# facebookresearch/holo_diffusion

Measured on AMD Instinct MI355X. Metric: denoise-steps/sec + rendered-rays/sec, 64^3x32 grid @400^2 render, higher is better.
Workload: dtype f32

## Files before the change

### holo_diffusion_amd/csrc/conv_weights.h

```cpp
#pragma once
#include <stddef.h>
#include <stdint.h>

#include "holo_knobs.h"

namespace holo {

int64_t conv_wino3_weight_floats(int CoutP, int CinP, int src_taps);

inline int64_t round64(int64_t n) { return (n + 63) & ~(int64_t)63; }

inline int conv_cout_tile(int Cout) { return Cout >= 64 ? 64 : 32; }
struct ConvWeightLayout {
  int Cout = 0, Cin = 0, taps = 0;
  int CoutP = 0, CinP = 0;
  int64_t f32_floats() const { return (int64_t)taps * CoutP * CinP; }
  int64_t bf16_elems() const { return 4 * round64(f32_floats()); }
  int64_t bft_offset() const { return 3 * f32_floats(); }
  int64_t wino2_floats() const { return (int64_t)(taps == 27 ? 48 : 4) * CoutP * CinP; }
  int64_t wino3_floats() const { return conv_wino3_weight_floats(CoutP, CinP, taps); }
};
inline ConvWeightLayout conv_weight_layout(int Cout, int Cin, int taps) {
  const int tile = conv_cout_tile(Cout);
  return {Cout, Cin, taps, (Cout + tile - 1) / tile * tile, (Cin + 31) / 32 * 32};
}

struct ConvCopies {
  bool bf16 = false, wino2 = false, wino3 = false;
};
inline ConvCopies forward_copies(const ConvWeightLayout& l, bool skip, const Knobs& k) {
  ConvCopies c;
  const bool c3 = l.taps == 27;
  c.bf16 = true;
  c.wino2 = k.conv_wino != 0 && (c3 || skip) && l.Cout <= 256 && l.Cin <= 768 && (l.Cout % 64 == 0 || (c3 && l.Cout == 32));
  c.wino3 = c.wino2 && k.conv_wino3 != 0 && l.Cout % 64 == 0;
  return c;
}
inline ConvCopies dgrad_copies(const ConvWeightLayout& l, int compute_mode, const Knobs& k) {
  ConvCopies c;
  c.wino2 = k.conv_wino != 0 && compute_mode == 0 && l.taps == 27 && l.Cout % 64 == 0 && l.Cout <= 768 && l.Cin <= 768;
  c.wino3 = c.wino2 && k.conv_wino3 != 0 && l.Cout <= 256;
  return c;
}

struct ConvWeights {
  float* f32 = nullptr;
  uint16_t* bf = nullptr;
  uint16_t* bft = nullptr;
  float* wino2 = nullptr;
  float* wino3 = nullptr;
  ConvWeightLayout layout;
};
int pack_conv_weights(const float* src_oidhw, const ConvWeights& dst, void* stream);

}
```

### holo_diffusion_amd/csrc/holo_kernels.h

```cpp
#pragma once
#include <stddef.h>
#include <stdint.h>

#include "../../include/holo_abi.h"
#include "conv_weights.h"
#include "holo_knobs.h"

struct HoloCtx {
  int device;
  int num_cus;
  int deterministic = 0;
};

namespace holo {

enum class ConvKernel : int32_t {
  Gather = 0,
  Halo = 1,
  RowTile = 2,
  Wino2 = 4,
  Bf16Wide = 5,
  Wino3 = 6,
  Stream1x1 = 7,
  Bf16Persistent = 8,
  S2Bf16 = 9,
  Qkv = 10,
  Bf16Stream1x1 = 11,
  Small1x1 = 12,
};

struct ConvParams {
  const float* src0;
  const float* src1;
  int C0, C1;
  int N, ID, IH, IW;
  int ups;
  int OD, OH, OW;
  int stride, pad, ksz;
  int Cout;
  const float* w;
  int CoutP, CinP;
  const float* coef;
  int act;
  const float* bias;
  const float* residual;
  float* out;
  const float* skip_src0;
  const float* skip_src1;
  int skip_C0, skip_C1;
  const float* skip_w;
  const uint16_t* w_bf;
// ... 11 lines not shown
  int stagger_ticks;
  unsigned long long* dbg;
  ConvKernel kernel;
  const float* w_wino2;
  const float* skip_w_wino2;
  const float* w_wino3;
  const float* skip_w_wino3;
  int wino3_up;
  const uint16_t* w_bft;
  const uint16_t* skip_w_bft;
  int in_bf16;
  int res_bf16;
  int out_bf16;
  uint16_t* qkv_q;
  uint16_t* qkv_k;
  uint16_t* qkv_vt;
  float qkv_scale;
  int qkv_T, qkv_CH, qkv_H;
  int qkv_sb, qkv_rows;
};

bool conv_s2_bf16_supported(const ConvParams& p);
int conv_s2_bf16_launch(const ConvParams& p, void* stream);

bool conv1x1_qkv_bf16_supported(const ConvParams& p);
void conv1x1_qkv_bf16_plan(ConvParams& p, int num_cus);
int conv1x1_qkv_bf16_launch(const ConvParams& p, void* stream);
bool conv1x1_bf16_stream_supported(const ConvParams& p);
void conv1x1_bf16_stream_plan(ConvParams& p, int num_cus);
int conv1x1_bf16_stream_slabs(const ConvParams& p);
int conv1x1_bf16_stream_launch(const ConvParams& p, void* stream);

int repack_conv_weight_wino3_launch(const float* w, float* out, int Cout, int Cin, int src_taps, int CoutP, int CinP,
                                    void* stream);
int conv_wino3_launch(const ConvParams& p, void* stream);
int conv_bf16p_launch(const ConvParams& p, void* stream);

size_t conv_plan(ConvParams& p, int num_cus, const Knobs& k, int plan_n = 0);
int conv_launch(const ConvParams& p, void* stream);
int conv_stats_slabs(const ConvParams& p);
double conv_flops(const ConvParams& p);
double conv_exec_flops(const ConvParams& p);

struct GemmParams {
  const float* A;
  const float* B;
// ... 395 lines not shown
```

### holo_diffusion_amd/csrc/holo_knobs.h

```cpp
#pragma once

#include <stdint.h>
#include <stdlib.h>

namespace holo {

#ifdef HOLO_EMU
constexpr bool EMU_BUILD = true;
#else
constexpr bool EMU_BUILD = false;
#endif

constexpr int64_t KNOB_UNSET = INT64_MIN;

#define HOLO_KNOBS(X)                                                                                                      \
  X(num_cus, "HOLO_NUM_CUS", POS, 0, CTX, "planners size grids and split-K for this many CUs (default: the device's)")     \
  X(conv_wino, "HOLO_CONV_WINO", INT, 1, HANDLE, "0: no Winograd copies of the conv weights (forward and dgrad)")          \
  X(conv_wino3, "HOLO_CONV_WINO3", INT, 1, HANDLE_PLAN, "0: no F(2x2x2, 3x3x3) copies / conv_wino3_kernel never chosen")   \
  X(keep_intermediates, "HOLO_KEEP_INTERMEDIATES", CH, '1', HANDLE,                                                        \
    "1: the plan releases no activation, holo_unet_fetch_block works")                                                     \
  X(render_v1, "HOLO_RENDER_V1", SET, 0, HANDLE, "the ray-per-column render kernel for everything")                        \
  X(render2_nw, "HOLO_RENDER2_NW", INT, 0, HANDLE, "8: the 8-wave form of render2_kernel's 12-wave configurations")        \
  X(render2_nrm_nw, "HOLO_RENDER2_NRM_NW", INT, 0, HANDLE,                                                                 \
    "8: rendered normals two waves per SIMD instead of 10 waves (the emulation build always runs 8)")                      \
  X(render_wgs, "HOLO_RENDER_WGS", POS, 0, HANDLE, "persistent render workgroups (default: one per CU)")                   \
  X(render_xcd, "HOLO_RENDER_XCD", RAW, KNOB_UNSET, HANDLE,                                                                \
    "XCD ranges of the render tile order (default 8; 2 in the emulation build; <= 1: plain order)")                        \
  X(render_tail, "HOLO_RENDER_TAIL", RAW, KNOB_UNSET, HANDLE,                                                              \
    "4-ray tiles at the end of every XCD range handed out as single rays (default: about two rounds; 3 in the "            \
    "emulation build; 0: off)")                                                                                            \
  X(render_static_tiles, "HOLO_RENDER_STATIC_TILES", SET, 0, HANDLE, "static tile stride instead of the dynamic hand-out") \
  X(render_timeline, "HOLO_RENDER_TIMELINE", SET, 0, HANDLE, "per-phase clocks of every render launch (synchronises!)")    \
  X(mlp_mean_bwd_chunk, "HOLO_MLP_MEAN_BWD_CHUNK", POS, 0, HANDLE,                                                         \
    "voxels per chunk of holo_mlp_mean_backward (default: what fits 4 GiB of rows; the emulation build: always 2048)")     \
  X(conv_wino_small, "HOLO_CONV_WINO_SMALL", INT, 1, PLAN, "0: under-filled levels take 64-voxel tiles, not Winograd")     \
  X(conv_force_tz2, "HOLO_CONV_FORCE_TZ2", INT, 0, PLAN, "1: 128-voxel tiles (hence the Winograd kernels) on small grids") \
  X(conv_qkv_fused, "HOLO_CONV_QKV_FUSED", INT, 1, PLAN, "0: row-tile qkv convolution + attn_pack_kernel")                 \
  X(conv1x1_bf16_stream, "HOLO_CONV1X1_BF16_STREAM", INT, 1, PLAN, "0: the row-tile kernel for bf16 1x1x1 convolutions")   \
  X(conv1x1_stream_min_m, "HOLO_CONV1X1_STREAM_MIN_M", INT, 131072, PLAN,                                                  \
    "rows from which a raw-input fp32 1x1x1 convolution streams (0: never)")                                               \
  X(conv1x1_small, "HOLO_CONV1X1_SMALL", INT, 1, PLAN, "0: the row-tile kernel for the fp32 attention's 1x1x1 convs")      \
  X(conv_s2t, "HOLO_CONV_S2T", INT, -1, PLAN, "stride-2 bf16 halo kernel: 0 never, 1 wherever defined (default: by fill)") \
  X(conv_bf16t, "HOLO_CONV_BF16T", INT, -1, PLAN, "bf16 wide-tile kernel: 0 never, 1 everywhere (default: by fill / K)")   \
  X(conv_bf16p, "HOLO_CONV_BF16P", INT, -1, PLAN,                                                                          \
    "its persistent form: 0 never, 1 every wide-tile launch, 2 activated input too (default: raw input)")                  \
  X(conv_bf16p_wgs, "HOLO_CONV_BF16P_WGS", INT, 0, PLAN, "at most this many persistent workgroups (0: no cap)")            \
  X(conv_wino3_min_items, "HOLO_CONV_WINO3_MIN_ITEMS", INT, KNOB_UNSET, PLAN,                                              \
    "work items from which conv_wino3_kernel runs (default: num_cus / 2)")                                                 \
  X(conv_wino3_up, "HOLO_CONV_WINO3_UP", INT, 1, PLAN,                                                                     \
    "0: upsampling convolutions on conv_wino3_kernel's generic form (64 pseudo-taps), not its 27-tap form")               \
  X(no_skip_fusion, "HOLO_NO_SKIP_FUSION", SET, 0, PLAN, "a ResBlock's 1x1x1 skip always as its own launch")               \
  X(skip_fusion_below_r, "HOLO_SKIP_FUSION_BELOW_R", RAW, 64, PLAN,                                                        \
    "exact fp32: the skip is fused into the second convolution below this grid edge")                                      \
  X(no_flash_attn, "HOLO_NO_FLASH_ATTN", SET, 0, PLAN, "attention as GEMM + softmax + GEMM")                               \
  X(bf16_flash_min_t, "HOLO_BF16_FLASH_MIN_T", RAW, 1024, PLAN, "tokens from which the bf16 mode takes its bf16 attention") \
  X(flash_split, "HOLO_FLASH_SPLIT", INT, 0, PLAN, "key splits of the fp32 attention, clamped to [1, T/128] (0: by fill)") \
  X(flash_v2_ksplit, "HOLO_FLASH_V2_KSPLIT", INT, 0, PLAN,                                                                 \
    "key splits of the bf16 attention: 1..8 dividing T into multiples of 128, else ignored")                               \
  X(attn_exact, "HOLO_ATTN_EXACT", SET, 0, PLAN, "bf16 attention: the exact loop alone, no LAZY pass")                     \
  X(debug_timestep_load, "HOLO_DEBUG_TIMESTEP_LOAD", INT, 0, PLAN, "how time_embed_kernel loads the timesteps (see it)")   \
  X(dgrad_s2_direct, "HOLO_DGRAD_S2_DIRECT", CH, '1', PLAN, "1: conv_dgrad_s2_kernel for every Downsample dgrad")          \
  X(wgrad_tiles, "HOLO_WGRAD_TILES", POS, 0, PLAN, "> 0: the tile weight-gradient kernel instead of the row-staged one")   \
  X(wgrad_reduce_tile_min, "HOLO_WGRAD_REDUCE_TILE_MIN", RAW, 1024, PLAN,                                                  \
    "64-element tiles from which the weight-gradient reduce runs its tile form")                                           \
  X(debug_plan, "HOLO_DEBUG_PLAN", SET, 0, PLAN, "[plan] lines on stderr: what every convolution / attention launches")    \
// ... 35 lines not shown
```

### holo_diffusion_amd/csrc/kernels_conv.hip

```cpp
#include <stdio.h>
#include <stdlib.h>

#include "holo_common.h"
#include "holo_kernels.h"

namespace holo {

namespace {

constexpr int BM = 128;
constexpr int BK = 32;
constexpr int LDK = 36;

__device__ __forceinline__ float silu_f(float v) { return v / (1.0f + __expf(-v)); }
__device__ __forceinline__ float silu_fast(float v) { return v * holo_rcp(1.0f + __expf(-v)); }

__device__ __forceinline__ float bf16_load(const uint16_t* p) { return __uint_as_float((uint32_t)(*p) << 16); }
__device__ __forceinline__ uint16_t bf16_round(float v) { return (uint16_t)(pack_bf16x2(v, 0.f) & 0xffffu); }
__device__ __forceinline__ float4 ld_act4(const float* base, int64_t idx, int bf) {
  if (bf) {
    const uint2 u = *reinterpret_cast<const uint2*>(reinterpret_cast<const uint16_t*>(base) + idx);
    return make_float4(__uint_as_float(u.x << 16), __uint_as_float(u.x & 0xffff0000u), __uint_as_float(u.y << 16),
                       __uint_as_float(u.y & 0xffff0000u));
  }
// ... 2230 lines not shown
    double* dst = stats + (((int64_t)n * gridDim.x + blockIdx.x) * Cout + c_base + tid * 4) * 2;
#pragma unroll
    for (int e = 0; e < 4; ++e) {
      dst[e * 2 + 0] = s[e];
      dst[e * 2 + 1] = s[4 + e];
    }
  }
}

const char* conv_kernel_name(ConvKernel k) {
  switch (k) {
    case ConvKernel::Gather: return "conv_igemm_kernel";
    case ConvKernel::Halo: return "conv_halo_kernel";
    case ConvKernel::RowTile: return "conv_small_kernel";
    case ConvKernel::Wino2: return "conv_wino2_kernel";
    case ConvKernel::Bf16Wide: return "conv_bf16t_kernel";
    case ConvKernel::Wino3: return "conv_wino3_kernel";
    case ConvKernel::Stream1x1: return "conv1x1_stream_kernel";
    case ConvKernel::Bf16Persistent: return "conv_bf16p_kernel";
    case ConvKernel::S2Bf16: return "conv_s2_bf16_kernel";
    case ConvKernel::Qkv: return "conv1x1_qkv_bf16_kernel";
    case ConvKernel::Bf16Stream1x1: return "conv1x1_bf16_stream_kernel";
    case ConvKernel::Small1x1: return "conv1x1_small_kernel";
  }
  return "?";
}

constexpr int SM_SPLIT_WGS_PER_CU = 2;
constexpr int BF16T_LONG_K = 192;
constexpr int BF16T_SPLIT_WGS_PER_CU_TOP = 2;
constexpr int BF16T_SPLIT_WGS_PER_CU = 1;

struct KSplit {
  int n, cps;
};
KSplit ksplit(int64_t want, int max_split, int chunks) {
  const int cps = (int)cdiv(chunks, want < max_split ? want : max_split);
  return {(int)cdiv(chunks, cps), cps};
}

bool conv1x1_small_supported(const ConvParams& p) {
  const int Cin = p.C0 + p.C1;
  const int64_t V = (int64_t)p.OD * p.OH * p.OW;
  return p.ksz == 1 && p.stride == 1 && p.pad == 0 && !p.ups && p.bf16 == 0 && !p.in_bf16 && !p.out_bf16 && !p.res_bf16 &&
         !p.skip_w && !p.src1 && p.C1 == 0 && !p.qkv_q && ((p.coef && !p.act) || p.residual) && (Cin % 32) == 0 &&
         Cin >= 32 && Cin <= 256 && p.CinP == Cin && (p.Cout % 64) == 0 && p.CoutP == p.Cout && p.ID == p.OD &&
// ... 11 lines not shown

size_t conv_plan(ConvParams& p, int num_cus, const Knobs& k, int plan_n) {
  const int Cin = p.C0 + p.C1;
  const int ncc = (Cin + BK - 1) / BK;
  const int nchunks = p.ksz * p.ksz * p.ksz * ncc;
  const int nsk = p.skip_w ? (int)cdiv(p.skip_C0 + p.skip_C1, BK) : 0;
  const int ncc16 = (Cin + 15) / 16;
  const int nsk16 = p.skip_w ? (p.skip_C0 + p.skip_C1 + 15) / 16 : 0;
  const int64_t M = (int64_t)p.N * p.OD * p.OH * p.OW;
  const int64_t Mc = (int64_t)(plan_n > 0 ? plan_n : p.N) * p.OD * p.OH * p.OW;
  const int bn = p.Cout >= 64 ? 64 : 32;
  const int64_t tiles = cdiv(Mc, BM) * cdiv(p.Cout, bn);
  const int64_t t8 = (Mc / 512) * cdiv(p.Cout, bn);
  const int64_t t3 = (Mc / 128) * (p.Cout / 64);
  const int64_t target = 2 * (int64_t)num_cus;
  const int64_t src_vox = (int64_t)p.ID * p.IH * p.IW;
  const int cmax = p.C0 > p.C1 ? p.C0 : p.C1;
  const int skmax = p.skip_C0 > p.skip_C1 ? p.skip_C0 : p.skip_C1;
  const bool fits32 = src_vox * (cmax > skmax ? cmax : skmax) * 4 < ((int64_t)1 << 32) &&
                      (int64_t)p.OD * p.OH * p.OW * p.Cout * 4 < ((int64_t)1 << 32);
  const bool halo = p.ksz == 3 && p.stride == 1 && p.pad == 1 && (p.OD % 2) == 0 && (p.OH % 8) == 0 && (p.OW % 8) == 0 &&
                    p.ID == p.OD && p.IH == p.OH && p.IW == p.OW && (Cin % 16) == 0 && fits32;
  const bool wino2_wide = p.w_wino2 && p.bf16 == 0 && p.Cout >= 64 && (p.Cout % 64) == 0 && (!p.skip_w || p.skip_w_wino2);
  const bool wino_small = k.conv_wino_small != 0 && wino2_wide && ncc >= 2;
  const int tz = tiles < target && k.conv_force_tz2 != 1 && !wino_small ? 1 : 2;

  const ConvKernel kernel = [&] {
    if (p.qkv_q) {
      if (k.conv_qkv_fused != 0 && conv1x1_qkv_bf16_supported(p)) return ConvKernel::Qkv;
      p.qkv_q = nullptr;
    }
    if (k.conv1x1_bf16_stream != 0 && conv1x1_bf16_stream_supported(p)) return ConvKernel::Bf16Stream1x1;
    if (!halo) {
      const int64_t min_m = k.conv1x1_stream_min_m;
      if (min_m > 0 && Mc >= min_m && p.ksz == 1 && p.stride == 1 && !p.ups && !p.coef && !p.residual && !p.skip_w && p.bf16 == 0 &&
          !p.in_bf16 && !p.out_bf16 && (p.Cout % 64) == 0 && (Cin % 32) == 0 && Cin >= 32 && Cin <= 256 &&
          (!p.src1 || (p.C0 % 32) == 0) && (Mc % 16) == 0 && p.ID == p.OD && p.IH == p.OH && p.IW == p.OW)
        return ConvKernel::Stream1x1;
      if (k.conv1x1_small != 0 && conv1x1_small_supported(p)) return ConvKernel::Small1x1;
      const int64_t s2t = k.conv_s2t;
      if (s2t != 0 && conv_s2_bf16_supported(p) && ((Mc / 128) * (p.Cout / 64) >= num_cus / 4 || s2t == 1))
        return ConvKernel::S2Bf16;
      return p.Cout >= 64 ? ConvKernel::RowTile : ConvKernel::Gather;
    }
    const int64_t bt = k.conv_bf16t;
    if (p.bf16 == 1 && p.in_bf16 && p.w_bft && (!p.skip_w || p.skip_w_bft) && (p.OD % 8) == 0 && (p.OH % 8) == 0 &&
        (p.OW % 8) == 0 && (p.Cout % 32) == 0 && (p.C0 % 8) == 0 && (p.skip_C0 % 8) == 0 && ((p.skip_C0 + p.skip_C1) % 8) == 0 &&
        (p.Cout >= 64 || !p.skip_w) && bt != 0 &&
        (t8 >= target || Cin + (p.skip_w ? p.skip_C0 + p.skip_C1 : 0) >= BF16T_LONG_K || bt == 1)) {
      const int64_t bp = k.conv_bf16p;
      const int wgs = num_cus & ~7;
      if (bp != 0 && (bp == 1 || bp == 2 || !p.coef) &&
          ((bf16t_split(p, t8, ncc16, num_cus).n == 1 && wgs >= 8 && t8 >= wgs) || bp == 1) &&
          (p.C1 == 0 || (p.C0 % 16) == 0) &&
          (!p.skip_w || (((p.skip_C0 + p.skip_C1) % 32) == 0 && (p.skip_C1 == 0 || (p.skip_C0 % 32) == 0))) &&
          src_vox < ((int64_t)1 << 24))
        return ConvKernel::Bf16Persistent;
      return ConvKernel::Bf16Wide;
    }
    if (tz == 2 && k.conv_wino3 != 0 && p.w_wino3 && p.bf16 == 0 && !p.in_bf16 && !p.out_bf16 && p.Cout >= 64 &&
        (p.Cout % 64) == 0 && (!p.skip_w || p.skip_w_wino3) && (p.OH % 8) == 0 && (p.OW % 8) == 0 && (p.OD % 2) == 0 &&
        (!p.coef || p.act) &&
        (int64_t)p.N * src_vox * (cmax > skmax ? cmax : skmax) * 4 < ((int64_t)1 << 32) &&
        (int64_t)wino3_split(t3, ncc, num_cus).n * Mc * p.Cout * 4 < ((int64_t)1 << 32) &&
        (!p.stats || (Mc / 128) * p.Cout * 16 < ((int64_t)1 << 32)) &&
        (!p.skip_w || ((p.skip_C0 % 16) == 0 && (p.skip_C1 % 4) == 0)) &&
        t3 * wino3_split(t3, ncc, num_cus).n >= (k.conv_wino3_min_items != KNOB_UNSET ? k.conv_wino3_min_items : num_cus / 2))
      return ConvKernel::Wino3;
    if (tz == 2 && (wino2_wide || (p.w_wino2 && p.bf16 == 0 && p.Cout == 32 && !p.skip_w))) return ConvKernel::Wino2;
    return ConvKernel::Halo;
  }();
  p.kernel = kernel;
  p.wino3_up = kernel == ConvKernel::Wino3 && p.ups && !p.coef && !p.skip_w && k.conv_wino3_up != 0 ? 1 : 0;

  switch (kernel) {
    case ConvKernel::Qkv:
    case ConvKernel::Bf16Stream1x1:
    case ConvKernel::Stream1x1:
    case ConvKernel::Small1x1:
      p.nsplit = 1;
      p.chunks_per_split = ncc;
      if (kernel == ConvKernel::Qkv) conv1x1_qkv_bf16_plan(p, num_cus);
      if (kernel == ConvKernel::Bf16Stream1x1) conv1x1_bf16_stream_plan(p, num_cus);
      break;
    case ConvKernel::S2Bf16:
      p.nsplit = 1;
      p.chunks_per_split = Cin / 16;
      break;
    case ConvKernel::RowTile: {
      const int64_t t2 = cdiv(Mc, SM_ROWS) * cdiv(p.Cout, 64);
      const int64_t tgt = SM_SPLIT_WGS_PER_CU * (int64_t)num_cus;
      const int nall = nchunks + nsk;
      const int max_split = nall / SG > 1 ? nall / SG : 1;
      const KSplit s = ksplit(t2 < tgt ? cdiv(tgt, t2) : 1, max_split, nall);
      p.nsplit = s.n;
      p.chunks_per_split = s.cps;
      break;
    }
    case ConvKernel::Gather: {
      const int max_split = nchunks / 4 > 1 ? nchunks / 4 : 1;
      const KSplit s = ksplit(tiles < target ? cdiv(target, tiles) : 1, max_split, nchunks);
      p.nsplit = s.n;
      p.chunks_per_split = s.cps;
      break;
    }
    case ConvKernel::Bf16Wide: {
      const KSplit s = bf16t_split(p, t8, ncc16, num_cus);
      p.tz = 8;
// ... 47 lines not shown
}

int conv_stats_slabs(const ConvParams& p) {
  const int64_t V = (int64_t)p.OD * p.OH * p.OW;
  if (p.nsplit > 1) {
    int B, vpb;
    gn_stats_geometry(p.Cout < 1024 ? p.Cout : 1024, V, &B, &vpb);
    return B;
  }
  switch (p.kernel) {
    case ConvKernel::Bf16Wide:
    case ConvKernel::Bf16Persistent:
      return (int)(V / 512);
    case ConvKernel::Halo:
      if (p.bf16 == 2 && p.w_bf && p.Cout >= 64 && !p.skip_w) return (int)(V / 32);
      [[fallthrough]];
    case ConvKernel::Wino2:
    case ConvKernel::Wino3:
      return (int)(V / (64 * p.tz)) * (p.Cout >= 64 ? 1 : 2);
    case ConvKernel::RowTile:
      return V % SM_ROWS == 0 ? (int)(V / SM_ROWS) : 0;
    case ConvKernel::S2Bf16:
      return (int)(V / 128);
    case ConvKernel::Bf16Stream1x1:
      return conv1x1_bf16_stream_slabs(p);
    case ConvKernel::Small1x1:
      return (int)(V / 16);
    default:
      return 0;
  }
}

double conv_flops(const ConvParams& p) {
  const double M = (double)p.N * p.OD * p.OH * p.OW;
  return 2.0 * M * p.Cout * ((double)(p.C0 + p.C1) * p.ksz * p.ksz * p.ksz + (p.skip_w ? p.skip_C0 + p.skip_C1 : 0));
}

double conv_exec_flops(const ConvParams& p) {
  const double wino3_taps = p.wino3_up ? 27.0 / 8.0 : 8.0;
  const double taps = p.kernel == ConvKernel::Wino3 ? wino3_taps : p.kernel == ConvKernel::Wino2 ? 12.0 : 0.0;
  if (taps == 0.0) return conv_flops(p);
  const double M = (double)p.N * p.OD * p.OH * p.OW;
  return 2.0 * M * p.Cout * ((double)(p.C0 + p.C1) * taps + (p.skip_w ? p.skip_C0 + p.skip_C1 : 0));
}

int conv_launch(const ConvParams& p, void* stream) {
// ... 137 lines not shown
      }
      dim3 g1((unsigned)(M / 16), (unsigned)(p.Cout / 64));
      switch (Cin / 32) {
        case 1: HOLO_LAUNCH(conv1x1_small_kernel<1>, g1, block, stream, p); break;
        case 2: HOLO_LAUNCH(conv1x1_small_kernel<2>, g1, block, stream, p); break;
        case 3: HOLO_LAUNCH(conv1x1_small_kernel<3>, g1, block, stream, p); break;
        case 4: HOLO_LAUNCH(conv1x1_small_kernel<4>, g1, block, stream, p); break;
        case 5: HOLO_LAUNCH(conv1x1_small_kernel<5>, g1, block, stream, p); break;
        case 6: HOLO_LAUNCH(conv1x1_small_kernel<6>, g1, block, stream, p); break;
        case 7: HOLO_LAUNCH(conv1x1_small_kernel<7>, g1, block, stream, p); break;
        case 8: HOLO_LAUNCH(conv1x1_small_kernel<8>, g1, block, stream, p); break;
        default:
          set_error("conv_launch: conv1x1_small_kernel: %d input channels", Cin);
          return -1;
      }
      break;
    }
    case ConvKernel::Bf16Persistent:
      if (conv_bf16p_launch(p, stream)) return -1;
      break;
    case ConvKernel::S2Bf16:
      if (conv_s2_bf16_launch(p, stream)) return -1;
      break;
    case ConvKernel::Qkv:
      if (conv1x1_qkv_bf16_launch(p, stream)) return -1;
      break;
    case ConvKernel::Bf16Stream1x1:
      if (conv1x1_bf16_stream_launch(p, stream)) return -1;
      break;
    default:
      set_error("conv_launch: unknown kernel %d", (int)p.kernel);
      return -1;
  }
  if (p.nsplit > 1) {
    const int64_t MC = M * p.Cout;
    const int64_t V = (int64_t)p.OD * p.OH * p.OW;
    int B, vpb;
    gn_stats_geometry(p.Cout < 1024 ? p.Cout : 1024, V, &B, &vpb);
    HOLO_LAUNCH(splitk_reduce_kernel, dim3((unsigned)B, (unsigned)p.N, (unsigned)cdiv(p.Cout, 1024)), dim3(256), stream,
                (const float*)p.partial,
                p.nsplit, MC, p.Cout, V, vpb, p.bias, p.skip_bias, p.residual, p.out, p.stats, p.res_bf16, p.out_bf16);
  }
  return 0;
}

}
// ... 1 lines not shown
```

### holo_diffusion_amd/csrc/kernels_conv_s2.hip

```cpp
#include "holo_common.h"
#include "holo_kernels.h"

namespace holo {
namespace {

constexpr int S2_HZ = 5, S2_HY = 17, S2_HX = 17, S2_XH = 9;
constexpr int S2_SLOTS = S2_HZ * S2_HY * 2 * S2_XH;
constexpr int S2_NV = S2_HZ * S2_HY * S2_HX;
constexpr int S2_IT = (2 * S2_NV + 255) / 256;

__global__ __launch_bounds__(256, 3) void conv_s2_bf16_kernel(ConvParams p) {
  __shared__ __attribute__((aligned(16))) float s_in[S2_SLOTS * 8];
  __shared__ float s_st[4 * 32 * 2];
  const int tid = threadIdx.x;
  const int lane = tid & 63;
  const int wave = tid >> 6;
  const int li = lane & 31;
  const int kg = lane >> 5;
  const int zw = wave >> 1;
  const int ch = wave & 1;
  const int Cin = p.C0;
  const int ncc = Cin / 16;
  const int ntx = p.OW >> 3, nty = p.OH >> 3, ntz = p.OD >> 1;
  int bt = blockIdx.x;
// ... 126 lines not shown
}

}

bool conv_s2_bf16_supported(const ConvParams& p) {
  const int Cin = p.C0 + p.C1;
  return p.ksz == 3 && p.stride == 2 && p.pad == 1 && !p.ups && p.bf16 == 1 && p.in_bf16 && p.out_bf16 && p.w_bft && !p.coef &&
         !p.residual && !p.skip_w && p.C1 == 0 && (Cin % 16) == 0 && (p.Cout % 64) == 0 && p.ID == 2 * p.OD && p.IH == 2 * p.OH &&
         p.IW == 2 * p.OW && (p.OD % 2) == 0 && (p.OH % 8) == 0 && (p.OW % 8) == 0 &&
         (int64_t)p.ID * p.IH * p.IW * Cin < ((int64_t)1 << 31);
}

int conv_s2_bf16_launch(const ConvParams& p, void* stream) {
  if (!conv_s2_bf16_supported(p) || p.nsplit != 1) {
    set_error("conv_s2_bf16_launch: unsupported launch (stride %d, %d -> %d channels, %d^3 -> %d^3)", p.stride, p.C0 + p.C1, p.Cout,
              p.ID, p.OD);
    return -1;
  }
  const int64_t tiles = (int64_t)p.N * (p.OD >> 1) * (p.OH >> 3) * (p.OW >> 3);
  HOLO_LAUNCH(conv_s2_bf16_kernel, dim3((unsigned)tiles, (unsigned)(p.Cout / 64)), dim3(256), stream, p);
  return 0;
}

}
```

### holo_diffusion_amd/csrc/unet_exec.cpp

```cpp
#include <math.h>
#include <stdarg.h>
#include <stdio.h>
#include <stdlib.h>
#include <string.h>

#include <functional>
#include <map>
#include <optional>
#include <string>
#include <vector>

#include "../../include/holo_abi.h"
#include "conv_weights.h"
#include "holo_common.h"
#include "holo_kernels.h"

namespace holo {

static thread_local char g_err[512] = "";
void set_error(const char* fmt, ...) {
  va_list ap;
  va_start(ap, fmt);
  vsnprintf(g_err, sizeof(g_err), fmt, ap);
  va_end(ap);
// ... 21 lines not shown
  if (!rc && dst.wino3) rc = repack_conv_weight_wino3_launch(src, dst.wino3, l.Cout, l.Cin, l.taps, l.CoutP, l.CinP, stream);
  return rc;
}


namespace {

enum BlockKind { B_CONV, B_RES, B_ATTN, B_DOWN, B_UP, B_HEAD };
struct Block {
  BlockKind kind;
  std::string prefix;
  int cin, cout;
};

enum ParamKind { P_PLAIN, P_CONV3, P_CONV1, P_EMB_W, P_EMB_B };

struct ParamSlot {
  std::string name;
  std::vector<int64_t> shape;
  int64_t numel;
  ParamKind kind;
  ConvWeights w;
  bool set;
  bool is_conv() const { return kind == P_CONV3 || kind == P_CONV1; }
  ConvWeightLayout layout(bool transposed = false) const {
    return conv_weight_layout((int)shape[transposed ? 1 : 0], (int)shape[transposed ? 0 : 1], kind == P_CONV3 ? 27 : 1);
  }
};
static bool is_downsample_weight(const std::string& name) {
  return name.size() > 10 && name.compare(name.size() - 10, 10, ".op.weight") == 0;
}

struct Arena {
  size_t top = 0, peak = 0;
  bool keep = false;
  std::vector<std::pair<size_t, size_t>> fl;
  static size_t al(size_t b) { return (b + 255) & ~(size_t)255; }
  size_t alloc(size_t bytes) {
    bytes = al(bytes);
    for (size_t i = 0; i < fl.size(); ++i) {
      if (fl[i].second >= bytes) {
        size_t off = fl[i].first;
        if (fl[i].second == bytes)
          fl.erase(fl.begin() + i);
        else {
          fl[i].first += bytes;
// ... 206 lines not shown
    for (int i = 0; i < c.num_res_blocks + 1; ++i) {
      const int ich = chans.back();
      chans.pop_back();
      std::vector<Block> layers;
      snprintf(buf, sizeof buf, "output_blocks.%d.0", oidx);
      layers.push_back(Block{B_RES, buf, ch + ich, mc * mult});
      ch = mc * mult;
      if (has_attn(ds)) {
        snprintf(buf, sizeof buf, "output_blocks.%d.%d", oidx, (int)layers.size());
        layers.push_back(Block{B_ATTN, buf, ch, ch});
      }
      if (level && i == c.num_res_blocks) {
        snprintf(buf, sizeof buf, "output_blocks.%d.%d", oidx, (int)layers.size());
        layers.push_back(Block{B_UP, buf, ch, ch});
        ds /= 2;
      }
      u->outputs.push_back(layers);
      ++oidx;
    }
  }
  u->final_ch = ch;
}

void add_param(HoloUnet* u, const std::string& name, std::vector<int64_t> shape, ParamKind kind) {
  ParamSlot s;
  s.name = name;
  s.shape = shape;
  s.numel = 1;
  for (auto d : shape) s.numel *= d;
  s.kind = kind;
  s.set = false;
  u->pindex[name] = (int)u->params.size();
  u->params.push_back(s);
}

void enumerate_params(HoloUnet* u) {
  const HoloUnetCfg& c = u->cfg;
  const int64_t mc = c.model_channels, ted = 4 * mc;
  u->ted = (int)ted;
  add_param(u, "time_embed.0.weight", {ted, mc}, P_PLAIN);
  add_param(u, "time_embed.0.bias", {ted}, P_PLAIN);
  add_param(u, "time_embed.2.weight", {ted, ted}, P_PLAIN);
  add_param(u, "time_embed.2.bias", {ted}, P_PLAIN);
  u->emb_rows = 0;
  auto add_block = [&](const Block& b) {
    const std::string& p = b.prefix;
    const int64_t ci = b.cin, co = b.cout;
    switch (b.kind) {
      case B_CONV:
// ... 11 lines not shown
        u->emb_rows += (int)(2 * co);
        add_param(u, p + ".out_layers.0.weight", {co}, P_PLAIN);
        add_param(u, p + ".out_layers.0.bias", {co}, P_PLAIN);
        add_param(u, p + ".out_layers.3.weight", {co, co, 3, 3, 3}, P_CONV3);
        add_param(u, p + ".out_layers.3.bias", {co}, P_PLAIN);
        if (ci != co) {
          add_param(u, p + ".skip_connection.weight", {co, ci, 1, 1, 1}, P_CONV1);
          add_param(u, p + ".skip_connection.bias", {co}, P_PLAIN);
        }
        break;
      case B_ATTN:
        add_param(u, p + ".norm.weight", {ci}, P_PLAIN);
        add_param(u, p + ".norm.bias", {ci}, P_PLAIN);
        add_param(u, p + ".qkv.weight", {3 * ci, ci, 1}, P_CONV1);
        add_param(u, p + ".qkv.bias", {3 * ci}, P_PLAIN);
        add_param(u, p + ".proj_out.weight", {ci, ci, 1}, P_CONV1);
        add_param(u, p + ".proj_out.bias", {ci}, P_PLAIN);
        break;
      case B_DOWN:
        add_param(u, p + ".op.weight", {co, ci, 3, 3, 3}, P_CONV3);
        add_param(u, p + ".op.bias", {co}, P_PLAIN);
        break;
      case B_UP:
        add_param(u, p + ".conv.weight", {co, ci, 3, 3, 3}, P_CONV3);
        add_param(u, p + ".conv.bias", {co}, P_PLAIN);
        break;
      case B_HEAD:
        break;
    }
  };
  for (auto& l : u->inputs)
    for (auto& b : l) add_block(b);
  for (auto& b : u->middle) add_block(b);
  for (auto& l : u->outputs)
    for (auto& b : l) add_block(b);
  add_param(u, "out.0.weight", {u->final_ch}, P_PLAIN);
  add_param(u, "out.0.bias", {u->final_ch}, P_PLAIN);
  add_param(u, "out.2.weight", {c.out_channels, u->final_ch, 3, 3, 3}, P_CONV3);
  add_param(u, "out.2.bias", {c.out_channels}, P_PLAIN);
}

struct StoreSizes {
  int64_t f32 = 0, bf = 0, wino = 0;
};
StoreSizes carve_params(HoloUnet* u, float* f32, uint16_t* bf, float* wino) {
  StoreSizes n;
  auto take = [](auto* base, int64_t& top, int64_t count) {
    auto* p = base ? base + top : nullptr;
    top += round64(count);
    return p;
  };
  for (ParamSlot& s : u->params) {
    if (s.kind == P_EMB_W || s.kind == P_EMB_B) continue;
    if (!s.is_conv()) {
      s.w.f32 = take(f32, n.f32, s.numel);
      continue;
    }
    const ConvWeightLayout l = s.w.layout = s.layout();
    const ConvCopies c = forward_copies(l, s.name.find("skip_connection") != std::string::npos, u->knobs);
    s.w.f32 = take(f32, n.f32, l.f32_floats());
    if (c.bf16) {
      s.w.bf = take(bf, n.bf, l.bf16_elems());
      s.w.bft = s.w.bf ? s.w.bf + l.bft_offset() : nullptr;
    }
    if (c.wino2) s.w.wino2 = take(wino, n.wino, l.wino2_floats());
    if (c.wino3) s.w.wino3 = take(wino, n.wino, l.wino3_floats());
  }
  u->emb_w = take(f32, n.f32, (int64_t)u->emb_rows * u->ted);
  u->emb_b = take(f32, n.f32, u->emb_rows);
  for (ParamSlot& s : u->params)
    if (f32 && (s.kind == P_EMB_W || s.kind == P_EMB_B)) {
      const int row = u->emb_row_off[s.name.substr(0, s.name.rfind(".emb_layers"))];
      s.w.f32 = s.kind == P_EMB_W ? u->emb_w + (int64_t)row * u->ted : u->emb_b + row;
    }
  return n;
}

ConvWeights W(const HoloUnet* u, const std::string& name) {
  auto it = u->pindex.find(name);
  return it == u->pindex.end() ? ConvWeights() : u->params[it->second].w;
}
const float* P(const HoloUnet* u, const std::string& name) { return W(u, name).f32; }
// ... 1770 lines not shown
```

### holo_diffusion_amd/unet.py

```python
from __future__ import annotations

import ctypes as C
import os
import math
from typing import Dict, Optional, Tuple

import torch

from . import _lib, runtime
from .registry import ReplaceableBase, apply_config, registry


class Unet3DBase(ReplaceableBase, torch.nn.Module):
    def forward(self, x: torch.Tensor, timesteps: torch.Tensor, cond_features: Optional[torch.Tensor] = None,
                **kwargs) -> torch.Tensor:
        raise NotImplementedError()


class _Node(torch.nn.Module):
    """Anonymous container used to reproduce the reference's dotted parameter names."""


def _add_param(root: torch.nn.Module, dotted: str, p: torch.nn.Parameter) -> None:
    parts = dotted.split(".")
# ... 362 lines not shown
        ws = runtime.workspace(self, dev, 0)
        dst = torch.empty(tuple(shape), device=dev)
        n = C.c_int64()
        _lib.check(L, L.holo_unet_fetch_block(self._handle, tag.encode(), runtime.ptr(dst), dst.numel(), C.byref(n),
                                              runtime.ptr(ws), runtime.stream_ptr(dev)), f"fetch_block {tag}")
        if n.value != dst.numel():
            raise _lib.HoloError(f"fetch_block {tag}: {n.value} elements, expected {dst.numel()}")
        return dst

    def time_convs(self, batch: int, iters: int, device: torch.device):
        h = self._ensure_handle(device)
        L = runtime.lib()
        nbytes = L.holo_unet_workspace_bytes(h, batch)
        ws = runtime.workspace(self, device, nbytes)
        ms, fl, nl = C.c_float(), C.c_double(), C.c_int()
        _lib.check(L, L.holo_unet_time_convs(h, batch, runtime.ptr(ws), ws.numel(), iters, runtime.stream_ptr(device),
                                             C.byref(ms), C.byref(fl), C.byref(nl)), "holo_unet_time_convs")
        return ms.value, fl.value, nl.value

    OP_NAMES = ("memset", "layout_in", "time_embed", "emb_linears", "gn_stats", "gn_finalize", "conv", "gemm",
                "softmax", "flash_attn", "layout_out")
    CONV_KERNELS = ("conv_igemm_kernel", "conv_halo_kernel", "conv_small_kernel", "conv_wino_kernel", "conv_wino2_kernel",
                    "conv_bf16t_kernel", "conv_wino3_kernel", "conv1x1_stream_kernel", "conv_bf16p_kernel", "conv_s2_bf16_kernel", "conv1x1_qkv_bf16_kernel", "conv1x1_bf16_stream_kernel",
                    "conv1x1_small_kernel")

    def time_ops(self, batch: int, iters: int, device: torch.device):
        h = self._ensure_handle(device)
        L = runtime.lib()
        nbytes = L.holo_unet_workspace_bytes(h, batch)
        ws = runtime.workspace(self, device, nbytes)
        R = getattr(self, "_handle_size", None) or self.image_size
        x = torch.randn(batch, self.in_channels, R, R, R, device=device)
        y = torch.empty(batch, self.out_channels, R, R, R, device=device)
        t = torch.full((batch,), 500, dtype=torch.int64, device=device)
        cap = 1024
        arr = (_lib.HoloOpTiming * cap)()
        n = C.c_int()
        _lib.check(L, L.holo_unet_time_ops(h, batch, runtime.ptr(x), runtime.ptr(t), runtime.ptr(y), runtime.ptr(ws),
                                           ws.numel(), iters, runtime.stream_ptr(device), arr, cap, C.byref(n)),
                   "holo_unet_time_ops")
        ops = []
        for i in range(min(n.value, cap)):
            a = arr[i]
            d = dict(op=self.OP_NAMES[a.op], ms=a.ms, flops=a.flops, flops_executed=a.flops_executed or a.flops, cin=a.cin,
                     cout=a.cout, out_dim=a.out_dim)
            if a.op == 6:
                d.update(kernel=self.CONV_KERNELS[a.kernel], tile_depth=a.tile_depth, fused_skip=bool(a.fused_skip),
# ... 32 lines not shown
```

Baseline: 169.4.

## Add exact-fp32 stride-2 halo conv kernel and widen Winograd-3 selection for upsample convs

Adds a new stride-2 3x3x3 fp32 MFMA kernel that stages a 9^3 halo brick in shared memory per 4^3 output tile and 64 output channels, with double-buffered register prefetch of the next channel slab. The planner selects it for downsampling convs when enough bricks fill the chip, instead of the row-tile or gather kernels. It also allocates Winograd F(2,3) copies for wide upsample conv weights and factors the wino3 eligibility test so that small, under-filled levels can pick 128-voxel Winograd tiles when wino3 fits. The cost is more weight memory, more kernel variants, and planner heuristics that may choose worse paths.

Measured after the change: 171.3 (median of 6 runs). 1.01x the previous value.

```diff
diff --git a/holo_diffusion_amd/csrc/conv_weights.h b/holo_diffusion_amd/csrc/conv_weights.h
--- a/holo_diffusion_amd/csrc/conv_weights.h
+++ b/holo_diffusion_amd/csrc/conv_weights.h
@@ -28,12 +28,13 @@
 struct ConvCopies {
   bool bf16 = false, wino2 = false, wino3 = false;
 };
-inline ConvCopies forward_copies(const ConvWeightLayout& l, bool skip, const Knobs& k) {
+inline ConvCopies forward_copies(const ConvWeightLayout& l, bool skip, bool upsample, const Knobs& k) {
   ConvCopies c;
   const bool c3 = l.taps == 27;
   c.bf16 = true;
   c.wino2 = k.conv_wino != 0 && (c3 || skip) && l.Cout <= 256 && l.Cin <= 768 && (l.Cout % 64 == 0 || (c3 && l.Cout == 32));
-  c.wino3 = c.wino2 && k.conv_wino3 != 0 && l.Cout % 64 == 0;
+  const bool up_wide = k.conv_wino != 0 && upsample && c3 && l.Cout <= 512 && l.Cin <= 768;
+  c.wino3 = (c.wino2 || up_wide) && k.conv_wino3 != 0 && l.Cout % 64 == 0;
   return c;
 }
 inline ConvCopies dgrad_copies(const ConvWeightLayout& l, int compute_mode, const Knobs& k) {
diff --git a/holo_diffusion_amd/csrc/holo_kernels.h b/holo_diffusion_amd/csrc/holo_kernels.h
--- a/holo_diffusion_amd/csrc/holo_kernels.h
+++ b/holo_diffusion_amd/csrc/holo_kernels.h
@@ -27,6 +27,7 @@
   Qkv = 10,
   Bf16Stream1x1 = 11,
   Small1x1 = 12,
+  S2Halo = 13,
 };
 
 struct ConvParams {
@@ -84,6 +85,8 @@
 
 bool conv_s2_bf16_supported(const ConvParams& p);
 int conv_s2_bf16_launch(const ConvParams& p, void* stream);
+bool conv_s2_halo_supported(const ConvParams& p);
+int conv_s2_halo_launch(const ConvParams& p, void* stream);
 
 bool conv1x1_qkv_bf16_supported(const ConvParams& p);
 void conv1x1_qkv_bf16_plan(ConvParams& p, int num_cus);
diff --git a/holo_diffusion_amd/csrc/holo_knobs.h b/holo_diffusion_amd/csrc/holo_knobs.h
--- a/holo_diffusion_amd/csrc/holo_knobs.h
+++ b/holo_diffusion_amd/csrc/holo_knobs.h
@@ -41,6 +41,8 @@
     "rows from which a raw-input fp32 1x1x1 convolution streams (0: never)")                                               \
   X(conv1x1_small, "HOLO_CONV1X1_SMALL", INT, 1, PLAN, "0: the row-tile kernel for the fp32 attention's 1x1x1 convs")      \
   X(conv_s2t, "HOLO_CONV_S2T", INT, -1, PLAN, "stride-2 bf16 halo kernel: 0 never, 1 wherever defined (default: by fill)") \
+  X(conv_s2_halo, "HOLO_CONV_S2_HALO", INT, -1, PLAN,                                                                      \
+    "stride-2 exact-fp32 halo kernel: 0 never, 1 wherever defined (default: where its bricks fill the chip un-split)")    \
   X(conv_bf16t, "HOLO_CONV_BF16T", INT, -1, PLAN, "bf16 wide-tile kernel: 0 never, 1 everywhere (default: by fill / K)")   \
   X(conv_bf16p, "HOLO_CONV_BF16P", INT, -1, PLAN,                                                                          \
     "its persistent form: 0 never, 1 every wide-tile launch, 2 activated input too (default: raw input)")                  \
diff --git a/holo_diffusion_amd/csrc/kernels_conv.hip b/holo_diffusion_amd/csrc/kernels_conv.hip
--- a/holo_diffusion_amd/csrc/kernels_conv.hip
+++ b/holo_diffusion_amd/csrc/kernels_conv.hip
@@ -2276,6 +2276,7 @@
     case ConvKernel::Qkv: return "conv1x1_qkv_bf16_kernel";
     case ConvKernel::Bf16Stream1x1: return "conv1x1_bf16_stream_kernel";
     case ConvKernel::Small1x1: return "conv1x1_small_kernel";
+    case ConvKernel::S2Halo: return "conv_s2_halo_kernel";
   }
   return "?";
 }
@@ -2333,7 +2334,16 @@
   const bool halo = p.ksz == 3 && p.stride == 1 && p.pad == 1 && (p.OD % 2) == 0 && (p.OH % 8) == 0 && (p.OW % 8) == 0 &&
                     p.ID == p.OD && p.IH == p.OH && p.IW == p.OW && (Cin % 16) == 0 && fits32;
   const bool wino2_wide = p.w_wino2 && p.bf16 == 0 && p.Cout >= 64 && (p.Cout % 64) == 0 && (!p.skip_w || p.skip_w_wino2);
-  const bool wino_small = k.conv_wino_small != 0 && wino2_wide && ncc >= 2;
+  const bool wino3_fit =
+      halo && k.conv_wino3 != 0 && p.w_wino3 && p.bf16 == 0 && !p.in_bf16 && !p.out_bf16 && p.Cout >= 64 && (p.Cout % 64) == 0 &&
+      (!p.skip_w || p.skip_w_wino3) && (p.OH % 8) == 0 && (p.OW % 8) == 0 && (p.OD % 2) == 0 &&
+      (!p.coef || p.act) &&
+      (int64_t)p.N * src_vox * (cmax > skmax ? cmax : skmax) * 4 < ((int64_t)1 << 32) &&
+      (int64_t)wino3_split(t3, ncc, num_cus).n * Mc * p.Cout * 4 < ((int64_t)1 << 32) &&
+      (!p.stats || (Mc / 128) * p.Cout * 16 < ((int64_t)1 << 32)) &&
+      (!p.skip_w || ((p.skip_C0 % 16) == 0 && (p.skip_C1 % 4) == 0)) &&
+      t3 * wino3_split(t3, ncc, num_cus).n >= (k.conv_wino3_min_items != KNOB_UNSET ? k.conv_wino3_min_items : num_cus / 2);
+  const bool wino_small = k.conv_wino_small != 0 && (wino2_wide || wino3_fit) && ncc >= 2;
   const int tz = tiles < target && k.conv_force_tz2 != 1 && !wino_small ? 1 : 2;
 
   const ConvKernel kernel = [&] {
@@ -2352,6 +2362,8 @@
       const int64_t s2t = k.conv_s2t;
       if (s2t != 0 && conv_s2_bf16_supported(p) && ((Mc / 128) * (p.Cout / 64) >= num_cus / 4 || s2t == 1))
         return ConvKernel::S2Bf16;
+      const int64_t s2h = k.conv_s2_halo;
+      if (s2h != 0 && conv_s2_halo_supported(p) && ((Mc / 64) * (p.Cout / 64) >= num_cus || s2h == 1)) return ConvKernel::S2Halo;
       return p.Cout >= 64 ? ConvKernel::RowTile : ConvKernel::Gather;
     }
     const int64_t bt = k.conv_bf16t;
@@ -2369,14 +2381,7 @@
         return ConvKernel::Bf16Persistent;
       return ConvKernel::Bf16Wide;
     }
-    if (tz == 2 && k.conv_wino3 != 0 && p.w_wino3 && p.bf16 == 0 && !p.in_bf16 && !p.out_bf16 && p.Cout >= 64 &&
-        (p.Cout % 64) == 0 && (!p.skip_w || p.skip_w_wino3) && (p.OH % 8) == 0 && (p.OW % 8) == 0 && (p.OD % 2) == 0 &&
-        (!p.coef || p.act) &&
-        (int64_t)p.N * src_vox * (cmax > skmax ? cmax : skmax) * 4 < ((int64_t)1 << 32) &&
-        (int64_t)wino3_split(t3, ncc, num_cus).n * Mc * p.Cout * 4 < ((int64_t)1 << 32) &&
-        (!p.stats || (Mc / 128) * p.Cout * 16 < ((int64_t)1 << 32)) &&
-        (!p.skip_w || ((p.skip_C0 % 16) == 0 && (p.skip_C1 % 4) == 0)) &&
-        t3 * wino3_split(t3, ncc, num_cus).n >= (k.conv_wino3_min_items != KNOB_UNSET ? k.conv_wino3_min_items : num_cus / 2))
+    if (tz == 2 && wino3_fit)
       return ConvKernel::Wino3;
     if (tz == 2 && (wino2_wide || (p.w_wino2 && p.bf16 == 0 && p.Cout == 32 && !p.skip_w))) return ConvKernel::Wino2;
     return ConvKernel::Halo;
@@ -2395,6 +2400,7 @@
       if (kernel == ConvKernel::Bf16Stream1x1) conv1x1_bf16_stream_plan(p, num_cus);
       break;
     case ConvKernel::S2Bf16:
+    case ConvKernel::S2Halo:
       p.nsplit = 1;
       p.chunks_per_split = Cin / 16;
       break;
@@ -2488,6 +2494,8 @@
       return V % SM_ROWS == 0 ? (int)(V / SM_ROWS) : 0;
     case ConvKernel::S2Bf16:
       return (int)(V / 128);
+    case ConvKernel::S2Halo:
+      return (int)(V / 64);
     case ConvKernel::Bf16Stream1x1:
       return conv1x1_bf16_stream_slabs(p);
     case ConvKernel::Small1x1:
@@ -2671,6 +2679,9 @@
     case ConvKernel::S2Bf16:
       if (conv_s2_bf16_launch(p, stream)) return -1;
       break;
+    case ConvKernel::S2Halo:
+      if (conv_s2_halo_launch(p, stream)) return -1;
+      break;
     case ConvKernel::Qkv:
       if (conv1x1_qkv_bf16_launch(p, stream)) return -1;
       break;
diff --git a/holo_diffusion_amd/csrc/kernels_conv_s2.hip b/holo_diffusion_amd/csrc/kernels_conv_s2.hip
--- a/holo_diffusion_amd/csrc/kernels_conv_s2.hip
+++ b/holo_diffusion_amd/csrc/kernels_conv_s2.hip
@@ -172,4 +172,185 @@
   return 0;
 }
 
-}
+
+namespace {
+
+constexpr int H2_H = 9;
+constexpr int H2_NV = H2_H * H2_H * H2_H;
+constexpr int H2_RP = 10;
+constexpr int H2_RS = 24;
+constexpr int H2_SLOTS = H2_H * H2_H * H2_RP;
+constexpr int H2_IT = (4 * H2_NV + 255) / 256;
+
+__global__ __launch_bounds__(256, 2) void conv_s2_halo_kernel(ConvParams p) {
+  __shared__ __attribute__((aligned(16))) float s_in[H2_SLOTS * H2_RS];
+  const int tid = threadIdx.x;
+  const int lane = tid & 63;
+  const int wave = tid >> 6;
+  const int lj = lane & 15;
+  const int kq = lane >> 4;
+  const int Cin = p.C0;
+  const int nsc = Cin / 16;
+  const int ntx = p.OW >> 2, nty = p.OH >> 2, ntz = p.OD >> 2;
+  int bt = blockIdx.x;
+  const int tx0 = (bt % ntx) << 2;
+  bt /= ntx;
+  const int ty0 = (bt % nty) << 2;
+  bt /= nty;
+  const int tz0 = (bt % ntz) << 2;
+  const int n = bt / ntz;
+  const int n0 = blockIdx.y * 64;
+
+  int goff[H2_IT], ldst[H2_IT];
+  unsigned okmask = 0, inmask = 0;
+#pragma unroll
+  for (int i = 0; i < H2_IT; ++i) {
+    const int id = tid + 256 * i;
+    const int v = min(id >> 2, H2_NV - 1), qd = id & 3;
+    const int hz = v / (H2_H * H2_H);
+    const int rem = v - hz * (H2_H * H2_H);
+    const int hy = rem / H2_H;
+    const int hx = rem - hy * H2_H;
+    int z = 2 * tz0 - 1 + hz, y = 2 * ty0 - 1 + hy, x = 2 * tx0 - 1 + hx;
+    const bool in = id < 4 * H2_NV;
+    const bool ok = in && z >= 0 && z < p.ID && y >= 0 && y < p.IH && x >= 0 && x < p.IW;
+    z = min(max(z, 0), p.ID - 1);
+    y = min(max(y, 0), p.IH - 1);
+    x = min(max(x, 0), p.IW - 1);
+    goff[i] = ((z * p.IH + y) * p.IW + x) * Cin + qd * 4;
+    ldst[i] = ((hz * H2_H + hy) * H2_RP + (hx & 1) * 5 + (hx >> 1)) * H2_RS + qd * 4;
+    okmask |= (ok ? 1u : 0u) << i;
+    inmask |= (in ? 1u : 0u) << i;
+  }
+  const float* src = p.src0 + (int64_t)n * p.ID * p.IH * p.IW * Cin;
+  float4 hreg[H2_IT];
+  auto issue = [&](int s) {
+#pragma unroll
+    for (int i = 0; i < H2_IT; ++i) hreg[i] = *reinterpret_cast<const float4*>(src + goff[i] + s * 16);
+  };
+  auto commit = [&]() {
+#pragma unroll
+    for (int i = 0; i < H2_IT; ++i) {
+      const bool keep = (okmask >> i) & 1u;
+      float4 v = hreg[i];
+      v.x = keep ? v.x : 0.f, v.y = keep ? v.y : 0.f, v.z = keep ? v.z : 0.f, v.w = keep ? v.w : 0.f;
+      if ((inmask >> i) & 1u) *reinterpret_cast<float4*>(s_in + ldst[i]) = v;
+    }
+  };
+
+  const int a_base = (2 * (lj >> 2) * H2_RP + (lj & 3)) * H2_RS + kq * 4;
+  auto load_a = [&](float4 (&a)[4], int tap) {
+    const int kd = tap / 9, kh = (tap - kd * 9) / 3, kw = tap - kd * 9 - kh * 3;
+    const int toff = ((kd * H2_H + kh) * H2_RP + (kw & 1) * 5 + (kw >> 1)) * H2_RS;
+#pragma unroll
+    for (int t = 0; t < 4; ++t) a[t] = *reinterpret_cast<const float4*>(s_in + a_base + toff + t * (2 * H2_H * H2_RP * H2_RS));
+  };
+  const int wncc = p.CinP / 32, wnsl = p.CoutP >> 4;
+  const float* w_lane = p.w + (int64_t)((n0 >> 4) + wave) * 512 + (kq & 1) * 256 + ((kq >> 1) * 16 + lj) * 4;
+  auto load_b = [&](int s, int tap) {
+    return *reinterpret_cast<const float4*>(w_lane + (int64_t)(tap * wncc + (s >> 1)) * wnsl * 512 + (s & 1) * 128);
+  };
+
+  f32x4 acc[4];
+#pragma unroll
+  for (int t = 0; t < 4; ++t)
+#pragma unroll
+    for (int r = 0; r < 4; ++r) acc[t][r] = 0.f;
+  const f32x4 zero4 = {0.f, 0.f, 0.f, 0.f};
+
+  float4 A[2][4], B[3];
+  issue(0);
+  B[0] = load_b(0, 0);
+  B[1] = load_b(0, 1);
+  commit();
+  __syncthreads();
+  for (int s = 0; s < nsc; ++s) {
+    const bool has_next = s + 1 < nsc;
+    if (has_next) issue(s + 1);
+    load_a(A[0], 0);
+    f32x4 blk[2][4];
+#pragma unroll
+    for (int tap = 0; tap < 27; ++tap) {
+      if (tap + 1 < 27) load_a(A[(tap + 1) & 1], tap + 1);
+      if (tap + 2 < 27) B[(tap + 2) % 3] = load_b(s, tap + 2);
+      __builtin_amdgcn_sched_barrier(0);
+      const float4(&a)[4] = A[tap & 1];
+      const float4& b = B[tap % 3];
+      const bool first = tap % 9 == 0;
+#pragma unroll
+      for (int t = 0; t < 4; ++t) blk[0][t] = __builtin_amdgcn_mfma_f32_16x16x4f32(a[t].x, b.x, first ? zero4 : blk[0][t], 0, 0, 0);
+#pragma unroll
+      for (int t = 0; t < 4; ++t) blk[1][t] = __builtin_amdgcn_mfma_f32_16x16x4f32(a[t].y, b.y, first ? zero4 : blk[1][t], 0, 0, 0);
+#pragma unroll
+      for (int t = 0; t < 4; ++t) blk[0][t] = __builtin_amdgcn_mfma_f32_16x16x4f32(a[t].z, b.z, blk[0][t], 0, 0, 0);
+#pragma unroll
+      for (int t = 0; t < 4; ++t) blk[1][t] = __builtin_amdgcn_mfma_f32_16x16x4f32(a[t].w, b.w, blk[1][t], 0, 0, 0);
+      if (tap % 9 == 8) {
+#pragma unroll
+        for (int t = 0; t < 4; ++t) acc[t] += blk[0][t] + blk[1][t];
+      }
+      __builtin_amdgcn_sched_barrier(0);
+    }
+    if (has_next) {
+      B[0] = load_b(s + 1, 0);
+      B[1] = load_b(s + 1, 1);
+    }
+    __syncthreads();
+    if (has_next) {
+      commit();
+      __syncthreads();
+    }
+  }
+
+  const int co = n0 + wave * 16 + lj;
+  const float bv = p.bias ? p.bias[co] : 0.f;
+  float* out = p.out + ((((int64_t)n * p.OD + tz0) * p.OH + ty0 + kq) * p.OW + tx0) * p.Cout + co;
+  float ssum = 0.f, ssq = 0.f;
+#pragma unroll
+  for (int t = 0; t < 4; ++t)
+#pragma unroll
+    for (int r = 0; r < 4; ++r) {
+      const float v = acc[t][r] + bv;
+      ssum += v;
+      ssq += v * v;
+      out[((int64_t)t * p.OH * p.OW + r) * p.Cout] = v;
+    }
+  if (p.stats) {
+    ssum += __shfl_xor(ssum, 16);
+    ssq += __shfl_xor(ssq, 16);
+    ssum += __shfl_xor(ssum, 32);
+    ssq += __shfl_xor(ssq, 32);
+    if (kq == 0) {
+      const int bricks_per_sample = ntx * nty * ntz;
+      const int slab = blockIdx.x % bricks_per_sample;
+      double2 rec;
+      rec.x = (double)ssum, rec.y = (double)ssq;
+      *reinterpret_cast<double2*>(p.stats + (((int64_t)n * bricks_per_sample + slab) * p.Cout + co) * 2) = rec;
+    }
+  }
+}
+
+}
+
+bool conv_s2_halo_supported(const ConvParams& p) {
+  const int Cin = p.C0 + p.C1;
+  return p.ksz == 3 && p.stride == 2 && p.pad == 1 && !p.ups && p.bf16 == 0 && !p.in_bf16 && !p.out_bf16 && !p.res_bf16 &&
+         !p.coef && !p.residual && !p.skip_w && !p.src1 && p.C1 == 0 && !p.qkv_q && (Cin % 32) == 0 && p.CinP == Cin &&
+         (p.Cout % 64) == 0 && p.CoutP == p.Cout && p.ID == 2 * p.OD && p.IH == 2 * p.OH && p.IW == 2 * p.OW &&
+         (p.OD % 4) == 0 && (p.OH % 4) == 0 && (p.OW % 4) == 0 &&
+         (int64_t)p.ID * p.IH * p.IW * Cin < ((int64_t)1 << 31) &&
+         (int64_t)p.N * (p.OD >> 2) * (p.OH >> 2) * (p.OW >> 2) < ((int64_t)1 << 31);
+}
+
+int conv_s2_halo_launch(const ConvParams& p, void* stream) {
+  if (!conv_s2_halo_supported(p) || p.nsplit != 1) {
+    set_error("conv_s2_halo_launch: unsupported launch (stride %d, %d -> %d channels, %d^3 -> %d^3)", p.stride, p.C0 + p.C1, p.Cout,
+              p.ID, p.OD);
+    return -1;
+  }
+  const int64_t bricks = (int64_t)p.N * (p.OD >> 2) * (p.OH >> 2) * (p.OW >> 2);
+  HOLO_LAUNCH(conv_s2_halo_kernel, dim3((unsigned)bricks, (unsigned)(p.Cout / 64)), dim3(256), stream, p);
+  return 0;
+}
+
+}
diff --git a/holo_diffusion_amd/csrc/unet_exec.cpp b/holo_diffusion_amd/csrc/unet_exec.cpp
--- a/holo_diffusion_amd/csrc/unet_exec.cpp
+++ b/holo_diffusion_amd/csrc/unet_exec.cpp
@@ -67,6 +67,7 @@
   ParamKind kind;
   ConvWeights w;
   bool set;
+  bool upsample = false;
   bool is_conv() const { return kind == P_CONV3 || kind == P_CONV1; }
   ConvWeightLayout layout(bool transposed = false) const {
     return conv_weight_layout((int)shape[transposed ? 1 : 0], (int)shape[transposed ? 0 : 1], kind == P_CONV3 ? 27 : 1);
@@ -319,9 +320,10 @@
   u->final_ch = ch;
 }
 
-void add_param(HoloUnet* u, const std::string& name, std::vector<int64_t> shape, ParamKind kind) {
+void add_param(HoloUnet* u, const std::string& name, std::vector<int64_t> shape, ParamKind kind, bool upsample = false) {
   ParamSlot s;
   s.name = name;
+  s.upsample = upsample;
   s.shape = shape;
   s.numel = 1;
   for (auto d : shape) s.numel *= d;
@@ -379,7 +381,7 @@
         add_param(u, p + ".op.bias", {co}, P_PLAIN);
         break;
       case B_UP:
-        add_param(u, p + ".conv.weight", {co, ci, 3, 3, 3}, P_CONV3);
+        add_param(u, p + ".conv.weight", {co, ci, 3, 3, 3}, P_CONV3, true);
         add_param(u, p + ".conv.bias", {co}, P_PLAIN);
         break;
       case B_HEAD:
@@ -414,7 +416,7 @@
       continue;
     }
     const ConvWeightLayout l = s.w.layout = s.layout();
-    const ConvCopies c = forward_copies(l, s.name.find("skip_connection") != std::string::npos, u->knobs);
+    const ConvCopies c = forward_copies(l, s.name.find("skip_connection") != std::string::npos, s.upsample, u->knobs);
     s.w.f32 = take(f32, n.f32, l.f32_floats());
     if (c.bf16) {
       s.w.bf = take(bf, n.bf, l.bf16_elems());
diff --git a/holo_diffusion_amd/unet.py b/holo_diffusion_amd/unet.py
--- a/holo_diffusion_amd/unet.py
+++ b/holo_diffusion_amd/unet.py
@@ -408,7 +408,7 @@
                 "softmax", "flash_attn", "layout_out")
     CONV_KERNELS = ("conv_igemm_kernel", "conv_halo_kernel", "conv_small_kernel", "conv_wino_kernel", "conv_wino2_kernel",
                     "conv_bf16t_kernel", "conv_wino3_kernel", "conv1x1_stream_kernel", "conv_bf16p_kernel", "conv_s2_bf16_kernel", "conv1x1_qkv_bf16_kernel", "conv1x1_bf16_stream_kernel",
-                    "conv1x1_small_kernel")
+                    "conv1x1_small_kernel", "conv_s2_halo_kernel")
 
     def time_ops(self, batch: int, iters: int, device: torch.device):
         h = self._ensure_handle(device)
```
